# yanzq95/DHD

Hardware: AMD Instinct MI355X
Metric: samples/sec (6-cam fwd+bwd) DHD-S view-transform hot path (higher is better)
Workload: dtype f32

## Files before the change

### dhd_amd/csrc/mghs_layout.h

```cpp
#pragma once
#include "vec16.h"

namespace dhd {

constexpr int kBlock = 256;
constexpr int kScanItems = 8;
constexpr int kChunk = kBlock * kScanItems;
constexpr int kTileC = 64;
constexpr int kCamFloats = 36;
#ifndef DHD_SEG_ROWS
#define DHD_SEG_ROWS 4
#endif
constexpr int kSegRows = DHD_SEG_ROWS;
constexpr int kSegMaxVox = 256 * kSegRows;
constexpr int kMaxTileX = 256;
constexpr int kRowGroup = 4;

struct Layout {
  int B, N, D, fh, fw, C, G;
  int dhw;
  int hw;
  int P;
  int V;
  int R;
  int n_chunks;
  int vox_base[DHD_MAX_GRIDS + 1];
  int row_base[DHD_MAX_GRIDS + 1];
  dhd_grid grid[DHD_MAX_GRIDS];
  int compact;
  int n_slots_max;
  int n_segs;
  int seg_base[DHD_MAX_GRIDS + 1];
  int nxc;
  int sched_heavy, sched_ratio;
  int flags;
  int columns;
  int* count;
  unsigned long long* scan_state;
  int* offset;
  int* key;
  int* rnk;
  int4* s_ent;
  float* cam;
  float* dg_part;
  float* fg_stage;
  float* vsum;
  int* nzoff;
  int* nzvox;
  int* p_slot;
  size_t zero_bytes;
};

inline size_t align_up(size_t v, size_t a) { return (v + a - 1) / a * a; }

__host__ __device__ inline int pt_natural(const Layout& L, int bn, int d, int h, int w) { return bn * L.dhw + (d * L.fh + h) * L.fw + w; }
__host__ __device__ inline int pt_index(const Layout& L, int bn, int d, int h, int w) {
#ifdef DHD_KEYS_ROWMAJOR
  return pt_natural(L, bn, d, h, w);
#else
  return bn * L.dhw + (d * L.fw + w) * L.fh + h;
#endif
}

inline int make_layout(const dhd_mghs_desc* d, const dhd_mghs_workspace* ws, Layout* L, size_t* state_bytes = nullptr,
                       size_t* scratch_bytes = nullptr) {
  if (!d) return DHD_EINVAL;
  if (d->batch <= 0 || d->n_cams <= 0 || d->n_depth <= 0 || d->fh <= 0 || d->fw <= 0 || d->channels <= 0)
    return DHD_EINVAL;
  if (d->n_grids < 1 || d->n_grids > DHD_MAX_GRIDS) return DHD_EINVAL;
  if (d->flags & ~(DHD_MGHS_DETERMINISTIC | DHD_MGHS_FEAT_GRAD_NCHW | DHD_MGHS_DEBUG_SCAN_SELF_SERVE)) return DHD_EINVAL;
  L->flags = d->flags;
  L->B = d->batch; L->N = d->n_cams; L->D = d->n_depth; L->fh = d->fh; L->fw = d->fw;
  L->C = d->channels; L->G = d->n_grids;
  L->hw = d->fh * d->fw;
  long dhw = (long)d->n_depth * L->hw;
  long P = (long)d->batch * d->n_cams * dhw;
  if (P > (1L << 29)) return DHD_EUNSUPPORTED;
  L->dhw = (int)dhw; L->P = (int)P;
  long v = 0, r = 0;
  bool compact = d->channels == kTileC;
  int nx_max = 0;
  for (int g = 0; g < DHD_MAX_GRIDS; ++g) {
    L->vox_base[g] = (int)v; L->row_base[g] = (int)r; L->seg_base[g] = (int)(r / kSegRows);
    if (g < d->n_grids) {
      const dhd_grid& gr = d->grid[g];
      if (gr.n[0] <= 0 || gr.n[1] <= 0 || gr.n[2] <= 0) return DHD_EINVAL;
      L->grid[g] = gr;
      v += (long)d->batch * gr.n[2] * gr.n[1] * gr.n[0];
      r += (long)d->batch * gr.n[2] * gr.n[1];
      if (v > (1L << 30)) return DHD_EUNSUPPORTED;
      compact = compact && gr.n[1] % kSegRows == 0 && gr.n[0] % 4 == 0 && gr.n[0] * kSegRows <= kSegMaxVox;
      nx_max = nx_max > gr.n[0] ? nx_max : gr.n[0];
    } else {
      L->grid[g] = d->grid[0];
    }
  }
  L->vox_base[DHD_MAX_GRIDS] = (int)v; L->row_base[DHD_MAX_GRIDS] = (int)r;
  for (int g = d->n_grids; g < DHD_MAX_GRIDS; ++g) { L->vox_base[g] = (int)v; L->row_base[g] = (int)r; }
  L->V = (int)v; L->R = (int)r;
  L->compact = compact ? 1 : 0;
  L->columns = (compact && d->n_grids > 1 && !(d->flags & DHD_MGHS_DETERMINISTIC) && d->fh == 32) ? 1 : 0;
  L->n_segs = compact ? (int)(r / kSegRows) : 0;
  for (int g = d->n_grids; g <= DHD_MAX_GRIDS; ++g) L->seg_base[g] = (int)(r / kSegRows);
  L->n_chunks = dhd_cdiv(v, kChunk);
  L->nxc = (nx_max + kMaxTileX - 1) / kMaxTileX;
  L->sched_heavy = 0; L->sched_ratio = 0;
  if (L->G > 1 && L->row_base[1] % kRowGroup == 0) {
    int heavy = L->row_base[1] / kRowGroup, light = (L->R - L->row_base[1]) / kRowGroup;
    int k = heavy > 0 ? light / heavy : 0;
    if (k > 4) k = 4;
    if (k == 3) k = 2;
    if (k == 1) k = 0;
    if (k >= 2) { L->sched_heavy = heavy; L->sched_ratio = k; }
  }
  if (ws) {
    if (!ws->state || !ws->scratch) return DHD_EINVAL;
    if ((reinterpret_cast<uintptr_t>(ws->state) | reinterpret_cast<uintptr_t>(ws->scratch)) & 255) return DHD_EINVAL;
  }
  const size_t P2 = 2 * (size_t)L->P;
  const size_t v0 = (size_t)L->vox_base[1], vb = (size_t)L->V - v0, pp = (size_t)L->P;
  const size_t max_slots = (v0 < pp ? v0 : pp) + (vb < pp ? vb : pp);
  L->n_slots_max = (int)max_slots;
  size_t off = 0;
  char* base = ws ? static_cast<char*>(ws->scratch) : nullptr;
  auto carve = [&](size_t n_words) { int* p = reinterpret_cast<int*>(base + off); off = align_up(off + n_words * 4, 256); return p; };
  L->count = carve((size_t)L->V);
  L->scan_state = reinterpret_cast<unsigned long long*>(carve(2 * (size_t)L->n_chunks));
  L->zero_bytes = off;
  if (compact) L->offset = carve((size_t)L->V + 1);
  L->key = carve(P2);
  L->rnk = carve(P2);
  if (compact) L->s_ent = reinterpret_cast<int4*>(carve(4 * P2));
  L->cam = reinterpret_cast<float*>(carve((size_t)L->B * L->N * kCamFloats));
  L->dg_part = reinterpret_cast<float*>(carve(compact ? 0 : P2));
  L->fg_stage = reinterpret_cast<float*>(carve(compact ? 0 : (size_t)L->B * L->N * L->hw * L->C));
  L->vsum = reinterpret_cast<float*>(carve(compact ? (max_slots + 1) * kTileC : 0));
  const size_t scratch_need = off;
  off = 0;
  base = ws ? static_cast<char*>(ws->state) : nullptr;
  L->nzoff = carve((size_t)L->V + 1);
  L->nzvox = carve(max_slots);
  L->p_slot = carve(P2);
  if (!compact) {
    L->offset = carve((size_t)L->V + 1);
    L->s_ent = reinterpret_cast<int4*>(carve(4 * P2));
  }
  const size_t state_need = off;
  if (state_bytes) *state_bytes = state_need;
  if (scratch_bytes) *scratch_bytes = scratch_need;
  if (ws && (ws->state_bytes < state_need || ws->scratch_bytes < scratch_need)) return DHD_ENOSPACE;
  return DHD_OK;
}

__device__ __forceinline__ int rfl(int v) { return __builtin_amdgcn_readfirstlane(v); }
__device__ __forceinline__ int lane_i(int v, int l) { return __builtin_amdgcn_readlane(v, l); }
__device__ __forceinline__ float lane_f(float v, int l) {
  return __int_as_float(__builtin_amdgcn_readlane(__float_as_int(v), l));
}
__device__ __forceinline__ int wave_sum_i(int v) {
  for (int m = 32; m > 0; m >>= 1) v += __shfl_xor(v, m, DHD_WAVE);
  return v;
}

struct OutPtrs { float* p[DHD_MAX_GRIDS]; long sb[DHD_MAX_GRIDS], sz[DHD_MAX_GRIDS], sc[DHD_MAX_GRIDS]; int dtype; };
struct InPtrs { const float* p[DHD_MAX_GRIDS]; long sb[DHD_MAX_GRIDS], sz[DHD_MAX_GRIDS], sc[DHD_MAX_GRIDS]; int dtype; };

template <class Ptrs, class T>
inline int make_views(const Layout& L, T* const bases[DHD_MAX_GRIDS], const dhd_tensor_view* views, Ptrs* o) {
  o->dtype = DHD_F32;
  if (views) {
    o->dtype = views[0].dtype;
    if (o->dtype != DHD_F32 && o->dtype != DHD_F16 && o->dtype != DHD_BF16) return DHD_EINVAL;
    if (o->dtype != DHD_F32 && !L.compact) return DHD_EUNSUPPORTED;
  }
  const long vec = o->dtype == DHD_F32 ? 4 : 8;
  for (int g = 0; g < DHD_MAX_GRIDS; ++g) {
    o->p[g] = nullptr; o->sb[g] = o->sz[g] = o->sc[g] = 0;
    if (g >= L.G) continue;
    const long plane = (long)L.grid[g].n[1] * L.grid[g].n[0];
    if (views) {
      if (!views[g].ptr) return DHD_EINVAL;
      o->p[g] = static_cast<T*>(const_cast<void*>(static_cast<const void*>(views[g].ptr)));
      o->sb[g] = views[g].batch_stride; o->sz[g] = views[g].z_stride; o->sc[g] = views[g].channel_stride;
      if (views[g].dtype != o->dtype) return DHD_EINVAL;
      if (((o->sb[g] | o->sz[g] | o->sc[g]) & (vec - 1)) || (reinterpret_cast<uintptr_t>(views[g].ptr) & 15)) return DHD_EINVAL;
      if (o->dtype != DHD_F32 && (L.grid[g].n[0] & 1)) return DHD_EUNSUPPORTED;
    } else {
      if (!bases || !bases[g]) return DHD_EINVAL;
      if (reinterpret_cast<uintptr_t>(bases[g]) & 15) return DHD_EINVAL;
      o->p[g] = bases[g];
      o->sb[g] = (long)L.grid[g].n[2] * L.C * plane; o->sz[g] = (long)L.C * plane; o->sc[g] = plane;
    }
  }
  return DHD_OK;
}

int launch_scan(const Layout& L, hipStream_t st);
int launch_stream_fwd(const Layout& L, const OutPtrs& o, int split, hipStream_t st, bool op = false);
int launch_stream_bwd(const Layout& L, const InPtrs& in, int split, hipStream_t st, bool op = false);

}
```

### dhd_amd/csrc/mghs_pool.hip

```cpp
#include "lift_device.h"
#include <stdlib.h>
#include "mghs_layout.h"

namespace dhd {
namespace {

#ifndef DHD_STREAM_BLOCK
#define DHD_STREAM_BLOCK 512
#endif
constexpr int kStreamBlock = DHD_STREAM_BLOCK;
constexpr int kStreamWaves = kStreamBlock / DHD_WAVE;
#ifndef DHD_TABLE_FLOATS
#define DHD_TABLE_FLOATS 8192
#endif
constexpr int kTableFloats = DHD_TABLE_FLOATS;

struct Segment {
  int g, b, z, y0, nx, ny, nz;
  int v0;
  int nvox;
};

__device__ __forceinline__ bool decode_segment(const Layout& L, int s, Segment* sg) {
  if (s >= L.n_segs) return false;
  int g = 0;
#pragma unroll
  for (int k = 1; k < DHD_MAX_GRIDS; ++k)
    if (k < L.G && s >= L.seg_base[k]) g = k;
  const dhd_grid& gr = L.grid[g];
  const int local = s - L.seg_base[g];
  const int per_plane = gr.n[1] / kSegRows;
  sg->g = g; sg->nx = gr.n[0]; sg->ny = gr.n[1]; sg->nz = gr.n[2];
  sg->y0 = (local % per_plane) * kSegRows;
  const int bz = local / per_plane;
  sg->z = bz % gr.n[2];
  sg->b = bz / gr.n[2];
  sg->nvox = kSegRows * gr.n[0];
  sg->v0 = L.vox_base[g] + local * sg->nvox;
  return true;
}

__device__ __forceinline__ int channels_per_pass(int nnz) {
  int cp = kTileC;
  while (cp > 4 && (nnz | 1) * cp > kTableFloats) cp >>= 1;
  return cp;
}

template <int J>
struct GatherStep {
  static __device__ __forceinline__ void load(float (&f)[DHD_WAVE], __amdgpu_buffer_rsrc_t feat_rsrc, int lane4, int pix,
                                              int jmax) {
    if ((J & 7) == 0 && J > jmax) return;
    f[J] = __int_as_float(__builtin_amdgcn_raw_buffer_load_b32(feat_rsrc, lane4, lane_i(pix, J) << 8, 0));
    GatherStep<J + 1>::load(f, feat_rsrc, lane4, pix, jmax);
  }
  static __device__ __forceinline__ void run(const float (&f)[DHD_WAVE], unsigned long long firsts, int term, int slot,
                                             float dv, float* vrow, int scratch_row, int jmax, int& cur, float& acc) {
    if ((J & 7) == 0 && J > jmax) return;
    if ((firsts >> J) & 1ull) {
      vrow[(size_t)cur * kTileC] = acc;
      cur = rfl((J == term) ? scratch_row : lane_i(slot, J));
      acc = 0.f;
    }
    acc = fmaf(lane_f(dv, J), f[J], acc);
    GatherStep<J + 1>::run(f, firsts, term, slot, dv, vrow, scratch_row, jmax, cur, acc);
  }
};
template <>
struct GatherStep<DHD_WAVE> {
  static __device__ __forceinline__ void load(float (&)[DHD_WAVE], __amdgpu_buffer_rsrc_t, int, int, int) {}
  static __device__ __forceinline__ void run(const float (&)[DHD_WAVE], unsigned long long, int, int, float, float*, int, int,
                                             int&, float&) {}
};

template <bool BANDS_ONLY>
__device__ __forceinline__ void gather_sums_body(const Layout& L, const float* __restrict__ depth, const float* __restrict__ feat,
                                                 const int block) {
  const int lane = threadIdx.x & 63;
  const int T0 = BANDS_ONLY ? L.offset[L.vox_base[1]] : 0;
  const int T = L.offset[L.V];
  const int per_xcd = ((T - T0 + kBlock - 1) / kBlock + 7) >> 3;
  if ((block >> 3) >= per_xcd) return;
  const int wg = (block & 7) * per_xcd + (block >> 3);
  const int a = rfl(T0 + (wg * (kBlock / DHD_WAVE) + (threadIdx.x >> 6)) * DHD_WAVE);
  if (a >= T) return;
  const int b = min(T, a + DHD_WAVE);
  const __amdgpu_buffer_rsrc_t feat_rsrc = __builtin_amdgcn_make_buffer_rsrc(
      const_cast<float*>(feat), 0, L.B * L.N * L.hw * kTileC * 4, 0x00020000);
  const int lane4 = 4 * lane;
  const int scratch_row = L.n_slots_max;
  float* vrow = L.vsum + lane;
  bool started = false;
  int cur = rfl(scratch_row);
  float acc = 0.f;
  int idx = a + lane;
  int slot_n = -1, prev_n = -2, pix_n = 0, pid_n = 0;
  float dv_n = 0.f;
  if (idx < T) {
    const int4 en = L.s_ent[idx];
    slot_n = en.z;
    pix_n = en.y;
    pid_n = en.x;
    if (idx > T0) prev_n = L.s_ent[idx - 1].z;
  }
  if (idx < T) dv_n = depth[pid_n];
  for (int a0 = a; a0 < T; a0 += DHD_WAVE) {
    const int nb = min(DHD_WAVE, T - a0);
    const int slot = slot_n, pix = pix_n;
    const float dv = dv_n;
    unsigned long long firsts = __ballot(lane < nb && slot != prev_n);
    int lo = 0;
    if (!started) {
      if (firsts == 0ull) lo = nb;
      else lo = __builtin_ctzll(firsts);
      if (a0 + lo >= b) break;
      started = lo < nb;
    }
    int term = DHD_WAVE;
    {
      const int s = min(max(b - a0, lo + 1), DHD_WAVE);
      const unsigned long long m = s >= DHD_WAVE ? 0ull : (firsts >> s) << s;
      if (m != 0ull) term = __builtin_ctzll(m);
      else if (nb < DHD_WAVE) term = nb;
    }
    const bool last = term < DHD_WAVE;
    if (last) firsts = (firsts & ((1ull << term) - 1ull)) | (1ull << term);
    if (lo >= nb) firsts = 0ull;
    idx = a0 + DHD_WAVE + lane;
    slot_n = -1; pix_n = 0; pid_n = 0;
    if (!last && idx < T) {
      const int4 en = L.s_ent[idx];
      slot_n = en.z;
      pix_n = en.y;
      pid_n = en.x;
      prev_n = L.s_ent[idx - 1].z;
    }
    if (lo < nb) {
      const int jmax = last ? term : DHD_WAVE - 1;
      float f[DHD_WAVE];
      GatherStep<0>::load(f, feat_rsrc, lane4, pix, jmax);
      GatherStep<0>::run(f, firsts, term, slot, dv, vrow, scratch_row, jmax, cur, acc);
    }
    if (last) { cur = rfl(scratch_row); break; }
    dv_n = 0.f;
    if (idx < T) dv_n = depth[pid_n];
  }
  vrow[(size_t)cur * kTileC] = acc;
}

template <bool BANDS_ONLY>
__global__ __launch_bounds__(kBlock) void mghs_gather_sums(Layout L, const float* __restrict__ depth,
                                                            const float* __restrict__ feat) {
  gather_sums_body<BANDS_ONLY>(L, depth, feat, (int)blockIdx.x);
}

constexpr int kDepthChunk = 8;

__global__ __launch_bounds__(kBlock) void mghs_zero_grid0_rows(Layout L) {
  const int n0 = L.nzoff[L.vox_base[1]];
  f32x4* v = reinterpret_cast<f32x4*>(L.vsum);
  const size_t n4 = (size_t)n0 * (kTileC / 4);
  const f32x4 z = {0.f, 0.f, 0.f, 0.f};
  for (size_t i = (size_t)blockIdx.x * kBlock + threadIdx.x; i < n4; i += (size_t)gridDim.x * kBlock) v[i] = z;
}

template <int FH, int H>
struct ColStep {
  static __device__ __forceinline__ void run(const float (&f)[FH], unsigned long long firsts, int slot, float dv, float* vrow,
                                             int& cur, float& acc) {
    if ((firsts >> H) & 1ull) {
      if (cur >= 0) atomicAdd(vrow + (size_t)cur * kTileC, acc);
      cur = rfl(lane_i(slot, H));
      acc = 0.f;
    }
    acc = fmaf(lane_f(dv, H), f[H], acc);
    ColStep<FH, H + 1>::run(f, firsts, slot, dv, vrow, cur, acc);
  }
};
template <int FH>
struct ColStep<FH, FH> {
  static __device__ __forceinline__ void run(const float (&)[FH], unsigned long long, int, float, float*, int&, float&) {}
};

template <int FH>
__device__ __forceinline__ void col_sums_body(const Layout& L, const float* __restrict__ depth, const float* __restrict__ feat,
                                              const int block) {
  const int lane = threadIdx.x & 63;
  const int n_chunks = (L.D + kDepthChunk - 1) / kDepthChunk;
  const int wave = rfl((int)(block * (kBlock / DHD_WAVE) + (threadIdx.x >> 6)));
  const int n_cols = L.B * L.N * L.fw;
  if (wave >= n_cols * n_chunks) return;
  const int chunk = wave / n_cols, col = wave - chunk * n_cols;
  const int bn = col / L.fw, w = col - bn * L.fw;
  float f[FH];
#pragma unroll
  for (int h = 0; h < FH; ++h) f[h] = feat[((size_t)(bn * FH + h) * L.fw + w) * kTileC + lane];
  float* vrow = L.vsum + lane;
  const int d0 = chunk * kDepthChunk;
  const int hl = lane < FH ? lane : FH - 1;
  int key[kDepthChunk], slot[kDepthChunk];
  float dv[kDepthChunk];
#pragma unroll
  for (int k = 0; k < kDepthChunk; ++k) {
    const int d = min(d0 + k, L.D - 1);
    const int p = ((bn * L.D + d) * FH + hl) * L.fw + w;
    key[k] = d0 + k < L.D ? L.key[pt_index(L, bn, d, hl, w)] : -1;
    dv[k] = depth[p];
  }
#pragma unroll
  for (int k = 0; k < kDepthChunk; ++k) slot[k] = key[k] >= 0 ? L.nzoff[key[k]] : -1;
#pragma unroll
  for (int k = 0; k < kDepthChunk; ++k) {
    const int prev = __shfl_up(slot[k], 1, DHD_WAVE);
    const unsigned long long firsts = __ballot(lane < FH && (lane == 0 || slot[k] != prev));
    const float dvk = key[k] >= 0 ? dv[k] : 0.f;
    int cur = -1;
    float acc = 0.f;
    ColStep<FH, 0>::run(f, firsts, slot[k], dvk, vrow, cur, acc);
    if (cur >= 0) atomicAdd(vrow + (size_t)cur * kTileC, acc);
  }
}

template <int FH>
__global__ __launch_bounds__(kBlock) void mghs_col_sums(Layout L, const float* __restrict__ depth, const float* __restrict__ feat) {
  col_sums_body<FH>(L, depth, feat, (int)blockIdx.x);
}

template <int FH>
__global__ __launch_bounds__(kBlock) void mghs_sums_cols_bands(Layout L, const float* __restrict__ depth, const float* __restrict__ feat,
                                                               int n_col_groups, int n_gather_groups, int kc) {
  const int grp = rfl((int)(blockIdx.x >> 3)), x = (int)(blockIdx.x & 7);
  const int period = grp / (kc + 1), r = grp - (kc + 1) * period;
  if (r < kc) {
    const int cg = kc * period + r;
    if (cg < n_col_groups) col_sums_body<FH>(L, depth, feat, (cg << 3) | x);
  } else if (period < n_gather_groups) {
    gather_sums_body<true>(L, depth, feat, (period << 3) | x);
  }
}

constexpr size_t kStreamLds = (size_t)kTableFloats * 4 + (size_t)kSegMaxVox * 2 + 16;

template <class T> __device__ __forceinline__ f32x4 pack_vox(const float* f) {
  typedef T vox __attribute__((ext_vector_type(kVec16<T>)));
  vox v;
#pragma unroll
  for (int k = 0; k < kVec16<T>; ++k) v[k] = (T)f[k];
  return __builtin_bit_cast(f32x4, v);
}
template <class T> __device__ __forceinline__ void unpack_vox(f32x4 v, float* f) { widen16<T>(__builtin_bit_cast(raw16<T>, v), f); }

template <class T, int OP = 0>
__global__ __launch_bounds__(kStreamBlock) void mghs_stream_fwd(Layout L, OutPtrs out, int split) {
  constexpr int VPL = kVec16<T>;
  extern __shared__ __attribute__((aligned(16))) char smem[];
  float* table = reinterpret_cast<float*>(smem);
  unsigned short* slot_of = reinterpret_cast<unsigned short*>(smem + (size_t)kTableFloats * 4);
  int* ctl = reinterpret_cast<int*>(smem + (size_t)kTableFloats * 4 + (size_t)kSegMaxVox * 2);

  const int seg = blockIdx.x / split, pw = kTileC / split;
  const int c_begin = (blockIdx.x % split) * pw, c_end = c_begin + pw;
  Segment sg;
  if (!decode_segment(L, seg, &sg)) return;
  const int t = threadIdx.x, lane = t & 63, wv = t >> 6;
  if (t == 0) ctl[0] = L.nzoff[sg.v0];
  if (t == 1) ctl[1] = L.nzoff[sg.v0 + sg.nvox];
  for (int i = t; i < kSegMaxVox / 2; i += kStreamBlock) reinterpret_cast<unsigned*>(slot_of)[i] = 0u;
  __syncthreads();
  const int k0 = rfl(ctl[0]), nnz = rfl(ctl[1]) - k0;
  for (int j = t; j < nnz; j += kStreamBlock) slot_of[L.nzvox[k0 + j] - sg.v0] = (unsigned short)(j + 1);
  const int cp = min(channels_per_pass(nnz), c_end - c_begin), pitch = nnz | 1;
  const int nvec = sg.nvox / VPL;
  T* og = reinterpret_cast<T*>(out.p[sg.g]);
  const long sb = out.sb[sg.g], sz = out.sz[sg.g], sc = out.sc[sg.g];
  for (int c_lo = c_begin; c_lo < c_end; c_lo += cp) {
    __syncthreads();
    for (int i = t; i < nnz * cp; i += kStreamBlock) {
      const int j = i / cp, cc = i % cp;
      table[cc * pitch + j] = L.vsum[(size_t)(k0 + j) * kTileC + c_lo + cc];
    }
    __syncthreads();
    T* base = og + (size_t)sg.b * sb + (size_t)sg.z * sz + (size_t)c_lo * sc + (size_t)sg.y0 * sg.nx;
    const int total = cp * nvec;
    constexpr int kStride = kStreamWaves * DHD_WAVE;
    const int q_step = kStride / nvec, r_step = kStride % nvec;
    int idx = wv * DHD_WAVE + lane;
    int cc = idx / nvec, i = idx % nvec;
    for (; idx < total; idx += kStride) {
      float f[VPL];
#pragma unroll
      for (int k = 0; k < VPL; ++k) f[k] = 0.f;
      unsigned sl[VPL / 2];
      if (VPL == 4) {
        const uint2 w = *reinterpret_cast<const uint2*>(slot_of + 4 * i);
        sl[0] = w.x; sl[1] = w.y;
      } else {
        const uint4 w = *reinterpret_cast<const uint4*>(slot_of + 8 * i);
        sl[0] = w.x; sl[1] = w.y; sl[VPL / 2 - 2] = w.z; sl[VPL / 2 - 1] = w.w;
      }
      unsigned any = 0;
#pragma unroll
      for (int k = 0; k < VPL / 2; ++k) any |= sl[k];
      if (any) {
#pragma unroll
        for (int k = 0; k < VPL / 2; ++k) {
          const unsigned s0 = sl[k] & 0xffffu, s1 = sl[k] >> 16;
          if (s0) f[2 * k] = table[cc * pitch + (s0 - 1)];
          if (s1) f[2 * k + 1] = table[cc * pitch + (s1 - 1)];
        }
      }
      f32x4* dst = reinterpret_cast<f32x4*>(base + (size_t)cc * sc) + i;
      __builtin_nontemporal_store(pack_vox<T>(f), dst);
      cc += q_step;
      i += r_step;
      if (i >= nvec) { i -= nvec; ++cc; }
    }
  }
}

template <class T, int OP = 0>
__global__ __launch_bounds__(kStreamBlock) void mghs_stream_bwd(Layout L, InPtrs og_in, int split) {
  constexpr int VPL = kVec16<T>;
  extern __shared__ __attribute__((aligned(16))) char smem[];
  float* table = reinterpret_cast<float*>(smem);
  unsigned short* slot_of = reinterpret_cast<unsigned short*>(smem + (size_t)kTableFloats * 4);
  int* ctl = reinterpret_cast<int*>(smem + (size_t)kTableFloats * 4 + (size_t)kSegMaxVox * 2);

  const int seg = blockIdx.x / split, pw = kTileC / split;
  const int c_begin = (blockIdx.x % split) * pw, c_end = c_begin + pw;
  Segment sg;
  if (!decode_segment(L, seg, &sg)) return;
  const int t = threadIdx.x, lane = t & 63, wv = t >> 6;
  if (t == 0) ctl[0] = L.nzoff[sg.v0];
  if (t == 1) ctl[1] = L.nzoff[sg.v0 + sg.nvox];
  for (int i = t; i < kSegMaxVox / 2; i += kStreamBlock) reinterpret_cast<unsigned*>(slot_of)[i] = 0u;
  __syncthreads();
  const int k0 = rfl(ctl[0]), nnz = rfl(ctl[1]) - k0;
  if (nnz == 0) return;
  for (int j = t; j < nnz; j += kStreamBlock) slot_of[L.nzvox[k0 + j] - sg.v0] = (unsigned short)(j + 1);
  const int cp = min(channels_per_pass(nnz), c_end - c_begin), pitch = nnz | 1;
  const int nvec = sg.nvox / VPL;
  const T* og = reinterpret_cast<const T*>(og_in.p[sg.g]);
  const long sb = og_in.sb[sg.g], sz = og_in.sz[sg.g], sc = og_in.sc[sg.g];
  constexpr int kStride = kStreamWaves * DHD_WAVE, kBatch = 5;
  const int q_step = kStride / nvec, r_step = kStride % nvec;
  const T* gbase = og + (size_t)sg.b * sb + (size_t)sg.z * sz + (size_t)sg.y0 * sg.nx;
  __syncthreads();
  for (int c_lo = c_begin; c_lo < c_end; c_lo += cp) {
    __syncthreads();
    const int total = cp * nvec;
    int idx = wv * DHD_WAVE + lane;
    int cc = idx / nvec, i = idx % nvec;
    for (; idx - lane < total; ) {
      unsigned sl[kBatch][VPL / 2], any[kBatch];
      f32x4 v[kBatch];
      int ccs[kBatch];
#pragma unroll
      for (int k = 0; k < kBatch; ++k) {
        const bool in = idx < total;
        if (VPL == 4) {
          const uint2 w = in ? *reinterpret_cast<const uint2*>(slot_of + 4 * i) : make_uint2(0u, 0u);
          sl[k][0] = w.x; sl[k][1] = w.y;
        } else {
          const uint4 w = in ? *reinterpret_cast<const uint4*>(slot_of + 8 * i) : make_uint4(0u, 0u, 0u, 0u);
          sl[k][0] = w.x; sl[k][1] = w.y; sl[k][VPL / 2 - 2] = w.z; sl[k][VPL / 2 - 1] = w.w;
        }
        any[k] = 0;
#pragma unroll
        for (int u = 0; u < VPL / 2; ++u) any[k] |= sl[k][u];
        ccs[k] = cc;
        const f32x4* p = any[k] ? reinterpret_cast<const f32x4*>(gbase + (size_t)(c_lo + cc) * sc) + i
                                  : reinterpret_cast<const f32x4*>(L.vsum);
        v[k] = __builtin_nontemporal_load(p);
        idx += kStride;
        cc += q_step;
        i += r_step;
        if (i >= nvec) { i -= nvec; ++cc; }
      }
#pragma unroll
      for (int k = 0; k < kBatch; ++k) {
        if (any[k]) {
          float f[VPL];
          unpack_vox<T>(v[k], f);
#pragma unroll
          for (int u = 0; u < VPL / 2; ++u) {
            const unsigned s0 = sl[k][u] & 0xffffu, s1 = sl[k][u] >> 16;
            if (s0) table[ccs[k] * pitch + (s0 - 1)] = f[2 * u];
            if (s1) table[ccs[k] * pitch + (s1 - 1)] = f[2 * u + 1];
          }
        }
      }
    }
    __syncthreads();
    for (int i = t; i < nnz * cp; i += kStreamBlock) {
      const int j = i / cp, cc = i % cp;
      L.vsum[(size_t)(k0 + j) * kTileC + c_lo + cc] = table[cc * pitch + j];
    }
  }
}

__device__ __forceinline__ float row16_sum(float v) {
  v += __int_as_float(__builtin_amdgcn_update_dpp(0, __float_as_int(v), 0x128, 0xf, 0xf, false));
  v += __int_as_float(__builtin_amdgcn_update_dpp(0, __float_as_int(v), 0x124, 0xf, 0xf, false));
  v += __int_as_float(__builtin_amdgcn_update_dpp(0, __float_as_int(v), 0x122, 0xf, 0xf, false));
  v += __int_as_float(__builtin_amdgcn_update_dpp(0, __float_as_int(v), 0x121, 0xf, 0xf, false));
  return v;
}

__global__ __launch_bounds__(kBlock) void mghs_pixel_bwd(Layout L, const float* __restrict__ depth,
                                                          const float* __restrict__ feat, float* __restrict__ depth_grad,
                                                          float* __restrict__ feat_grad) {
  const int lane = threadIdx.x & 63;
  const int es = lane >> 4, cq = lane & 15;
  const int per_xcd = gridDim.x >> 3;
  const int wg = (blockIdx.x & 7) * per_xcd + (blockIdx.x >> 3);
  const int q = rfl(wg * (kBlock / DHD_WAVE) + (threadIdx.x >> 6));
  if (q >= L.B * L.N * L.hw) return;
  const int bn = q / L.hw, pl = q % L.hw;
  const int p0 = bn * L.dhw + pl;
  const f32x4 f = reinterpret_cast<const f32x4*>(feat)[(size_t)q * (kTileC / 4) + cq];
  const f32x4* gc = reinterpret_cast<const f32x4*>(L.vsum) + cq;
  f32x4 fg = {0.f, 0.f, 0.f, 0.f};
  const int n_cand = 2 * L.D;
  constexpr int kRounds = DHD_WAVE / 4, kU = 8;
  for (int e0 = 0; e0 < n_cand; e0 += DHD_WAVE) {
    const int nb = min(DHD_WAVE, n_cand - e0);
    int slot = -1;
    float dv = 0.f;
    if (lane < nb) {
      const int e = e0 + lane;
      const int pid = p0 + (e >> 1) * L.hw;
      slot = L.p_slot[(e & 1) * L.P + pid];
      dv = depth[pid];
    }
    float mine = 0.f;
#pragma unroll
    for (int u0 = 0; u0 < kRounds; u0 += kU) {
      if (4 * u0 >= nb) break;
      f32x4 g[kU];
      float d[kU];
#pragma unroll
      for (int j = 0; j < kU; ++j) {
        const int i = 4 * (u0 + j) + es;
        const int sl = __shfl(slot, i, DHD_WAVE);
        d[j] = __shfl(dv, i, DHD_WAVE);
        g[j] = sl >= 0 ? gc[(size_t)sl * (kTileC / 4)] : fg * 0.f;
      }
#pragma unroll
      for (int j = 0; j < kU; ++j) {
        fg += g[j] * d[j];
        const float part = row16_sum((g[j].x * f.x + g[j].y * f.y) + (g[j].z * f.z + g[j].w * f.w));
        const float both = part + __shfl_xor(part, 16, DHD_WAVE);
        if (cq == u0 + j) mine = both;
      }
    }
    const int cand = 4 * cq + es;
    if (!(es & 1) && cand < nb) depth_grad[p0 + ((e0 + cand) >> 1) * L.hw] = mine;
  }
#pragma unroll
  for (int c = 0; c < 4; ++c) {
    float v = fg[c];
    v += __shfl_xor(v, 16, DHD_WAVE);
    v += __shfl_xor(v, 32, DHD_WAVE);
    fg[c] = v;
  }
  if (es == 0) {
    if (L.flags & DHD_MGHS_FEAT_GRAD_NCHW) {
      float* dst = feat_grad + ((size_t)bn * kTileC + 4 * cq) * L.hw + pl;
#pragma unroll
      for (int c = 0; c < 4; ++c) dst[(size_t)c * L.hw] = fg[c];
    } else {
      reinterpret_cast<f32x4*>(feat_grad)[(size_t)q * (kTileC / 4) + cq] = fg;
    }
  }
}

__global__ __launch_bounds__(kLiftBlock) void mghs_fg_to_nchw(const float* __restrict__ src, float* __restrict__ dst, int rows, int cols) {
  __shared__ float tile[64][65];
  transpose_tile(tile, src, dst, rows, cols, blockIdx.z, blockIdx.y * 64, blockIdx.x * 64);
}

__global__ __launch_bounds__(kBlock) void mghs_sum_parts(const float* __restrict__ part, int P, float* __restrict__ out) {
  const int i = blockIdx.x * kBlock + threadIdx.x;
  if (i < P) out[i] = part[i] + part[P + i];
}

constexpr int kRowBlock = 512;
constexpr int kRowWaves = kRowBlock / DHD_WAVE;

struct RowTile {
  int g, b, z, y, nx, ny, nz;
  int vrow;
};

__device__ __forceinline__ bool decode_row(const Layout& L, int r, RowTile* t) {
  if (r >= L.R) return false;
  int g = 0;
#pragma unroll
  for (int k = 1; k < DHD_MAX_GRIDS; ++k)
    if (k < L.G && r >= L.row_base[k]) g = k;
  const dhd_grid& gr = L.grid[g];
  int local = r - L.row_base[g];
  t->g = g; t->nx = gr.n[0]; t->ny = gr.n[1]; t->nz = gr.n[2];
  t->y = local % gr.n[1];
  int bz = local / gr.n[1];
  t->z = bz % gr.n[2];
  t->b = bz / gr.n[2];
  t->vrow = L.vox_base[g] + local * gr.n[0];
  return true;
}

__device__ __forceinline__ int scheduled_tile(const Layout& L, int block, int* xchunk) {
  const int pos = xcd_grouped_tile(block, kRowGroup * L.nxc);
  *xchunk = pos % L.nxc;
  const int rpos = pos / L.nxc;
  int grp = rpos / kRowGroup;
  const int within = rpos % kRowGroup;
  if (L.sched_heavy > 0) {
    const int k1 = L.sched_ratio + 1;
    if (grp < L.sched_heavy * k1) {
      const int q = grp / k1, r = grp % k1;
      grp = (r == 0) ? q : L.sched_heavy + q * L.sched_ratio + (r - 1);
    }
  }
  return grp * kRowGroup + within;
}

__global__ __launch_bounds__(kRowBlock) void mghs_rows_fwd(Layout L, const float* __restrict__ depth,
                                                           const float* __restrict__ feat, OutPtrs out, int tile_stride) {
  extern __shared__ __attribute__((aligned(16))) char smem[];
  float* tile = reinterpret_cast<float*>(smem);
  int* offs = reinterpret_cast<int*>(smem + (size_t)kTileC * tile_stride * 4);
  RowTile rt;
  int xchunk;
  if (!decode_row(L, scheduled_tile(L, blockIdx.x, &xchunk), &rt)) return;
  const int c0 = blockIdx.y * kTileC;
  const int cn = min(kTileC, L.C - c0);
  const int x0 = xchunk * kMaxTileX;
  if (x0 >= rt.nx) return;
  const int xn = min(kMaxTileX, rt.nx - x0);
  const int t = threadIdx.x, lane = t & 63, wv = t >> 6;

  for (int i = t; i <= xn; i += kRowBlock) offs[i] = L.offset[rt.vrow + x0 + i];
  for (int i = t; i < cn * tile_stride; i += kRowBlock) tile[i] = 0.f;
  __syncthreads();

  if (offs[xn] != offs[0]) {
    const int CL = next_pow2(cn);
    const int nsub = DHD_WAVE / CL;
    const int c = lane % CL, sub = lane / CL;
    const bool c_ok = c < cn;
    const float* featc = feat + c0 + c;
    for (int x = wv; x < xn; x += kRowWaves) {
      const int s = offs[x], e = offs[x + 1];
      if (e == s) continue;
      float acc = 0.f;
      for (int s0 = s; s0 < e; s0 += DHD_WAVE) {
        const int nb = min(DHD_WAVE, e - s0);
        int pix = 0;
        float dv = 0.f;
        if (lane < nb) {
          const int4 en = L.s_ent[s0 + lane];
          pix = en.y;
          dv = depth[en.x];
        }
        const int steps = (nb + nsub - 1) / nsub;
        for (int k = 0; k < steps; ++k) {
          const int i = k * nsub + sub;
          const bool live = i < nb;
          int q = __shfl(pix, live ? i : 0, DHD_WAVE);
          float d = __shfl(dv, live ? i : 0, DHD_WAVE);
          float f = (live && c_ok) ? featc[(size_t)q * L.C] : 0.f;
          acc = fmaf(d, f, acc);
        }
      }
      for (int m = CL; m < DHD_WAVE; m <<= 1) acc += __shfl_xor(acc, m, DHD_WAVE);
      if (sub == 0 && c_ok) tile[c * tile_stride + x] = acc;
    }
    __syncthreads();
  }

  float* og = out.p[rt.g];
  const bool vec = ((rt.nx & 3) == 0) && ((xn & 3) == 0) && ((x0 & 3) == 0);
  for (int cc = wv; cc < cn; cc += kRowWaves) {
    size_t row = (size_t)rt.b * out.sb[rt.g] + (size_t)rt.z * out.sz[rt.g] + (size_t)(c0 + cc) * out.sc[rt.g] + (size_t)rt.y * rt.nx + x0;
    const float* src = tile + cc * tile_stride;
    if (vec) {
      f32x4* dst = reinterpret_cast<f32x4*>(og + row);
      for (int i = lane; i < xn / 4; i += DHD_WAVE) {
        f32x4 v = {src[4 * i], src[4 * i + 1], src[4 * i + 2], src[4 * i + 3]};
        __builtin_nontemporal_store(v, dst + i);
      }
    } else {
      for (int i = lane; i < xn; i += DHD_WAVE) __builtin_nontemporal_store(src[i], og + row + i);
    }
  }
}

__global__ __launch_bounds__(kRowBlock) void mghs_rows_bwd(Layout L, const float* __restrict__ depth,
                                                           const float* __restrict__ feat, InPtrs og,
                                                           float* __restrict__ feat_grad, int tile_stride) {
  extern __shared__ __attribute__((aligned(16))) char smem[];
  float* tile = reinterpret_cast<float*>(smem);
  int* offs = reinterpret_cast<int*>(smem + (size_t)kTileC * tile_stride * 4);
  RowTile rt;
  int xchunk;
  if (!decode_row(L, scheduled_tile(L, blockIdx.x, &xchunk), &rt)) return;
  const int c0 = blockIdx.y * kTileC;
  const int cn = min(kTileC, L.C - c0);
  const int x0 = xchunk * kMaxTileX;
  if (x0 >= rt.nx) return;
  const int xn = min(kMaxTileX, rt.nx - x0);
  const int t = threadIdx.x, lane = t & 63, wv = t >> 6;

  for (int i = t; i <= xn; i += kRowBlock) offs[i] = L.offset[rt.vrow + x0 + i];
  __syncthreads();
  if (offs[xn] == offs[0]) return;

  const float* gsrc = og.p[rt.g];
  const bool vec = ((rt.nx & 3) == 0) && ((xn & 3) == 0) && ((x0 & 3) == 0);
  for (int cc = wv; cc < cn; cc += kRowWaves) {
    size_t row = (size_t)rt.b * og.sb[rt.g] + (size_t)rt.z * og.sz[rt.g] + (size_t)(c0 + cc) * og.sc[rt.g] + (size_t)rt.y * rt.nx + x0;
    float* dst = tile + cc * tile_stride;
    if (vec) {
      const float4* src = reinterpret_cast<const float4*>(gsrc + row);
      for (int i = lane; i < xn / 4; i += DHD_WAVE) {
        float4 v = src[i];
        dst[4 * i] = v.x; dst[4 * i + 1] = v.y; dst[4 * i + 2] = v.z; dst[4 * i + 3] = v.w;
      }
    } else {
      for (int i = lane; i < xn; i += DHD_WAVE) dst[i] = gsrc[row + i];
    }
  }
  __syncthreads();

  float* dgp = L.dg_part + (rt.g == 0 ? 0 : L.P);
  const bool dg_atomic = L.C > kTileC;
  const int CL = next_pow2(cn);
  const int nsub = DHD_WAVE / CL;
  const int c = lane % CL, sub = lane / CL;
  const bool c_ok = c < cn;
  const float* featc = feat + c0 + c;
  float* fgc = feat_grad + c0 + c;
  for (int x = wv; x < xn; x += kRowWaves) {
    const int s = offs[x], e = offs[x + 1];
    if (e == s) continue;
    const float g = c_ok ? tile[c * tile_stride + x] : 0.f;
    for (int s0 = s; s0 < e; s0 += DHD_WAVE) {
      const int nb = min(DHD_WAVE, e - s0);
      int pix = 0, pid = 0;
      float dv = 0.f;
      if (lane < nb) {
        const int4 en = L.s_ent[s0 + lane];
        pix = en.y;
        pid = en.x;
        dv = depth[pid];
      }
      float mine = 0.f;
      const int steps = (nb + nsub - 1) / nsub;
      for (int k = 0; k < steps; ++k) {
        const int i = k * nsub + sub;
        const bool live = i < nb;
        int q = __shfl(pix, live ? i : 0, DHD_WAVE);
        float d = __shfl(dv, live ? i : 0, DHD_WAVE);
        float prod = 0.f;
        if (live && c_ok) {
          float f = featc[(size_t)q * L.C];
          unsafeAtomicAdd(fgc + (size_t)q * L.C, g * d);
          prod = g * f;
        }
        float tot = group_sum(prod, CL);
        int owner_sub = lane - k * nsub;
        float got = __shfl(tot, (owner_sub >= 0 && owner_sub < nsub) ? owner_sub * CL : 0, DHD_WAVE);
        if (owner_sub >= 0 && owner_sub < nsub) mine = got;
      }
      if (lane < nb) {
        if (dg_atomic) unsafeAtomicAdd(dgp + pid, mine); else dgp[pid] = mine;
      }
    }
  }
}

void rows_launch_shape(const Layout& L, int* stride, size_t* smem, dim3* grid) {
  int nx_max = 0;
  for (int g = 0; g < L.G; ++g) nx_max = nx_max > L.grid[g].n[0] ? nx_max : L.grid[g].n[0];
  int xt = nx_max < kMaxTileX ? nx_max : kMaxTileX;
  *stride = xt | 1;
  *smem = (size_t)kTileC * (*stride) * 4 + (size_t)(kMaxTileX + 1) * 4;
  *grid = dim3(xcd_grouped_blocks(L.R * L.nxc, kRowGroup * L.nxc), dhd_cdiv(L.C, kTileC), 1);
}

}

int launch_stream_fwd(const Layout& L, const OutPtrs& o, int split, hipStream_t st, bool op) {
  if (!L.compact || L.n_segs <= 0) return DHD_EINVAL;
  if (op) {
    if (o.dtype != DHD_F32) return DHD_EUNSUPPORTED;
    hipLaunchKernelGGL((mghs_stream_fwd<float, 1>), dim3(L.n_segs * split), dim3(kStreamBlock), kStreamLds, st, L, o, split);
    DHD_LAUNCH_CHECK();
    return DHD_OK;
  }
  return with_dtype<NativeHalf>(o.dtype, [&](auto* t) {
    hipLaunchKernelGGL(mghs_stream_fwd<std::remove_pointer_t<decltype(t)>>, dim3(L.n_segs * split), dim3(kStreamBlock), kStreamLds, st, L, o, split);
    DHD_LAUNCH_CHECK();
    return DHD_OK;
  });
}

int launch_stream_bwd(const Layout& L, const InPtrs& in, int split, hipStream_t st, bool op) {
  if (!L.compact || L.n_segs <= 0) return DHD_EINVAL;
  if (op) {
    if (in.dtype != DHD_F32) return DHD_EUNSUPPORTED;
    hipLaunchKernelGGL((mghs_stream_bwd<float, 1>), dim3(L.n_segs * split), dim3(kStreamBlock), kStreamLds, st, L, in, split);
    DHD_LAUNCH_CHECK();
    return DHD_OK;
  }
  return with_dtype<NativeHalf>(in.dtype, [&](auto* t) {
    hipLaunchKernelGGL(mghs_stream_bwd<std::remove_pointer_t<decltype(t)>>, dim3(L.n_segs * split), dim3(kStreamBlock), kStreamLds, st, L, in, split);
    DHD_LAUNCH_CHECK();
    return DHD_OK;
  });
}

}

using namespace dhd;

static int stream_split(const Layout& L) {
  return (long)L.P < 300L * L.n_segs ? 4 : 2;
}

extern "C" {

int dhd_mghs_forward_gather(const dhd_mghs_desc* desc, const float* depth, const float* feat_nhwc, const dhd_mghs_workspace* workspace,
                            void* stream) {
  Layout L;
  int rc = make_layout(desc, workspace, &L);
  if (rc) return rc;
  if (!workspace || !depth || !feat_nhwc) return DHD_EINVAL;
  if (L.compact && !dhd_aligned(16, feat_nhwc)) return DHD_EINVAL;
  if (!L.compact) return DHD_OK;
  hipStream_t st = dhd_stream(stream);
  if (L.columns) {
    hipLaunchKernelGGL(mghs_zero_grid0_rows, dim3(1024), dim3(kBlock), 0, st, L);
    const int waves = L.B * L.N * L.fw * dhd_cdiv(L.D, kDepthChunk);
    const dim3 grid(dhd_cdiv(waves, kBlock / DHD_WAVE));
    const int n_gather = dhd_cdiv((long)L.P, 8 * kBlock) * 8;
    static const bool merged = getenv("DHD_MGHS_SEPARATE_SUMS") == nullptr;
    constexpr int kc = 2;
    if (merged) {
      const int ncg = dhd_cdiv(grid.x, 8), ngg = n_gather / 8;
      const int periods = ((ncg + kc - 1) / kc) > ngg ? (ncg + kc - 1) / kc : ngg;
      hipLaunchKernelGGL(mghs_sums_cols_bands<32>, dim3(periods * (kc + 1) * 8), dim3(kBlock), 0, st, L, depth, feat_nhwc, ncg, ngg, kc);
    } else {
      hipLaunchKernelGGL(mghs_col_sums<32>, grid, dim3(kBlock), 0, st, L, depth, feat_nhwc);
      hipLaunchKernelGGL(mghs_gather_sums<true>, dim3(n_gather), dim3(kBlock), 0, st, L, depth, feat_nhwc);
    }
  } else {
    hipLaunchKernelGGL(mghs_gather_sums<false>, dim3(dhd_cdiv(2L * L.P, 8 * kBlock) * 8), dim3(kBlock), 0, st, L, depth, feat_nhwc);
  }
  DHD_LAUNCH_CHECK();
  return DHD_OK;
}

static int forward_stream_impl(const dhd_mghs_desc* desc, const float* depth, const float* feat_nhwc,
                               float* const out[DHD_MAX_GRIDS], const dhd_tensor_view* views, const dhd_mghs_workspace* workspace,
                               void* stream) {
  Layout L;
  int rc = make_layout(desc, workspace, &L);
  if (rc) return rc;
  if (!workspace || !depth || !feat_nhwc || (!out && !views)) return DHD_EINVAL;
  if (L.compact && !dhd_aligned(16, feat_nhwc)) return DHD_EINVAL;
  OutPtrs o;
  if ((rc = make_views<OutPtrs, float>(L, out, views, &o))) return rc;
  hipStream_t st = dhd_stream(stream);
  if (L.compact) {
    if ((rc = launch_stream_fwd(L, o, o.dtype == DHD_F32 ? stream_split(L) : 2, st))) return rc;
  } else {
    int stride; size_t smem; dim3 grid;
    rows_launch_shape(L, &stride, &smem, &grid);
    hipLaunchKernelGGL(mghs_rows_fwd, grid, dim3(kRowBlock), smem, st, L, depth, feat_nhwc, o, stride);
    DHD_LAUNCH_CHECK();
  }
  return DHD_OK;
}

int dhd_mghs_forward_stream(const dhd_mghs_desc* desc, const float* depth, const float* feat_nhwc,
                            float* const out[DHD_MAX_GRIDS], const dhd_mghs_workspace* workspace, void* stream) {
  return forward_stream_impl(desc, depth, feat_nhwc, out, nullptr, workspace, stream);
}

int dhd_mghs_forward_stream_views(const dhd_mghs_desc* desc, const float* depth, const float* feat_nhwc,
                                  const dhd_tensor_view out[DHD_MAX_GRIDS], const dhd_mghs_workspace* workspace, void* stream) {
  if (!out) return DHD_EINVAL;
  return forward_stream_impl(desc, depth, feat_nhwc, nullptr, out, workspace, stream);
}

int dhd_mghs_forward(const dhd_mghs_desc* desc, const float* depth, const float* feat_nhwc,
                     float* const out[DHD_MAX_GRIDS], const dhd_mghs_workspace* workspace, void* stream) {
  int rc = dhd_mghs_forward_gather(desc, depth, feat_nhwc, workspace, stream);
  if (rc) return rc;
  return forward_stream_impl(desc, depth, feat_nhwc, out, nullptr, workspace, stream);
}

int dhd_mghs_forward_views(const dhd_mghs_desc* desc, const float* depth, const float* feat_nhwc,
                           const dhd_tensor_view out[DHD_MAX_GRIDS], const dhd_mghs_workspace* workspace, void* stream) {
  if (!out) return DHD_EINVAL;
  int rc = dhd_mghs_forward_gather(desc, depth, feat_nhwc, workspace, stream);
  if (rc) return rc;
  return forward_stream_impl(desc, depth, feat_nhwc, nullptr, out, workspace, stream);
}

static int backward_impl(const dhd_mghs_desc* desc, const float* depth, const float* feat_nhwc,
                         const float* const out_grad[DHD_MAX_GRIDS], const dhd_tensor_view* views, float* depth_grad,
                         float* feat_grad_nhwc, const dhd_mghs_workspace* workspace, void* stream) {
  Layout L;
  int rc = make_layout(desc, workspace, &L);
  if (rc) return rc;
  if (!workspace || !depth || !feat_nhwc || (!out_grad && !views) || !depth_grad || !feat_grad_nhwc) return DHD_EINVAL;
  if (L.compact && !dhd_aligned(16, feat_nhwc, feat_grad_nhwc)) return DHD_EINVAL;
  InPtrs in;
  if ((rc = make_views<InPtrs, const float>(L, out_grad, views, &in))) return rc;
  hipStream_t st = dhd_stream(stream);
  if (L.compact) {
    if ((rc = launch_stream_bwd(L, in, stream_split(L) == 2 ? 2 : 1, st))) return rc;
    hipLaunchKernelGGL(mghs_pixel_bwd, dim3(dhd_cdiv((long)L.B * L.N * L.hw, 8 * (kBlock / DHD_WAVE)) * 8), dim3(kBlock), 0, st, L,
                       depth, feat_nhwc, depth_grad, feat_grad_nhwc);
    DHD_LAUNCH_CHECK();
    return DHD_OK;
  }
  const bool to_nchw = (L.flags & DHD_MGHS_FEAT_GRAD_NCHW) != 0;
  float* fg = to_nchw ? L.fg_stage : feat_grad_nhwc;
  DHD_HIP(hipMemsetAsync(L.dg_part, 0, 2 * (size_t)L.P * 4, st));
  DHD_HIP(hipMemsetAsync(fg, 0, (size_t)L.B * L.N * L.hw * L.C * 4, st));
  int stride; size_t smem; dim3 grid;
  rows_launch_shape(L, &stride, &smem, &grid);
  hipLaunchKernelGGL(mghs_rows_bwd, grid, dim3(kRowBlock), smem, st, L, depth, feat_nhwc, in, fg, stride);
  DHD_LAUNCH_CHECK();
  if (to_nchw) {
    hipLaunchKernelGGL(mghs_fg_to_nchw, dim3(dhd_cdiv(L.C, 64), dhd_cdiv(L.hw, 64), L.B * L.N), dim3(kLiftBlock), 0, st, fg,
                       feat_grad_nhwc, L.hw, L.C);
    DHD_LAUNCH_CHECK();
  }
  hipLaunchKernelGGL(mghs_sum_parts, dim3(dhd_cdiv(L.P, kBlock)), dim3(kBlock), 0, st, L.dg_part, L.P, depth_grad);
  DHD_LAUNCH_CHECK();
  return DHD_OK;
}

int dhd_mghs_backward(const dhd_mghs_desc* desc, const float* depth, const float* feat_nhwc,
                      const float* const out_grad[DHD_MAX_GRIDS], float* depth_grad, float* feat_grad_nhwc,
                      const dhd_mghs_workspace* workspace, void* stream) {
  return backward_impl(desc, depth, feat_nhwc, out_grad, nullptr, depth_grad, feat_grad_nhwc, workspace, stream);
}

int dhd_mghs_backward_views(const dhd_mghs_desc* desc, const float* depth, const float* feat_nhwc,
                            const dhd_tensor_view out_grad[DHD_MAX_GRIDS], float* depth_grad, float* feat_grad_nhwc,
                            const dhd_mghs_workspace* workspace, void* stream) {
  if (!out_grad) return DHD_EINVAL;
  return backward_impl(desc, depth, feat_nhwc, nullptr, out_grad, depth_grad, feat_grad_nhwc, workspace, stream);
}

}
```

Measured before the change: 2768.

## Overlap band-grid streaming with grid-0 gather sums in a merged forward kernel

Adds a by-grid forward path. It first gathers band-grid sums, then runs one merged kernel whose workgroups are split proportionally between streaming the band segments and computing grid-0 gather sums. A final launch streams the grid-0 segments. The goal is to overlap the two independent phases and avoid a full serial gather-then-stream dependency. The gather inner loop can also load features in two halves to lower register pressure in the merged kernel. This adds a third launch and mixed-role workgroups that may cut occupancy because of the stream kernel's LDS use. The path is on by default but is not used when the columns path is active.

```diff
diff --git a/dhd_amd/csrc/mghs_layout.h b/dhd_amd/csrc/mghs_layout.h
--- a/dhd_amd/csrc/mghs_layout.h
+++ b/dhd_amd/csrc/mghs_layout.h
@@ -62,6 +62,16 @@
 #endif
 }
 
+struct RoleSlot { int point, index; };
+__host__ __device__ inline RoleSlot role_of_group(int g, int n_stream, int n_point) {
+  const long long n = (long long)n_stream + n_point;
+  const int before = (int)((long long)g * n_point / n), upto = (int)((long long)(g + 1) * n_point / n);
+  RoleSlot r;
+  r.point = upto > before ? 1 : 0;
+  r.index = r.point ? before : g - before;
+  return r;
+}
+
 inline int make_layout(const dhd_mghs_desc* d, const dhd_mghs_workspace* ws, Layout* L, size_t* state_bytes = nullptr,
                        size_t* scratch_bytes = nullptr) {
   if (!d) return DHD_EINVAL;
diff --git a/dhd_amd/csrc/mghs_pool.hip b/dhd_amd/csrc/mghs_pool.hip
--- a/dhd_amd/csrc/mghs_pool.hip
+++ b/dhd_amd/csrc/mghs_pool.hip
@@ -46,15 +46,15 @@
   return cp;
 }
 
-template <int J>
+template <int J, int END, int N>
 struct GatherStep {
-  static __device__ __forceinline__ void load(float (&f)[DHD_WAVE], __amdgpu_buffer_rsrc_t feat_rsrc, int lane4, int pix,
+  static __device__ __forceinline__ void load(float (&f)[N], __amdgpu_buffer_rsrc_t feat_rsrc, int lane4, int pix,
                                               int jmax) {
     if ((J & 7) == 0 && J > jmax) return;
-    f[J] = __int_as_float(__builtin_amdgcn_raw_buffer_load_b32(feat_rsrc, lane4, lane_i(pix, J) << 8, 0));
-    GatherStep<J + 1>::load(f, feat_rsrc, lane4, pix, jmax);
-  }
-  static __device__ __forceinline__ void run(const float (&f)[DHD_WAVE], unsigned long long firsts, int term, int slot,
+    f[J & (N - 1)] = __int_as_float(__builtin_amdgcn_raw_buffer_load_b32(feat_rsrc, lane4, lane_i(pix, J) << 8, 0));
+    GatherStep<J + 1, END, N>::load(f, feat_rsrc, lane4, pix, jmax);
+  }
+  static __device__ __forceinline__ void run(const float (&f)[N], unsigned long long firsts, int term, int slot,
                                              float dv, float* vrow, int scratch_row, int jmax, int& cur, float& acc) {
     if ((J & 7) == 0 && J > jmax) return;
     if ((firsts >> J) & 1ull) {
@@ -62,27 +62,28 @@
       cur = rfl((J == term) ? scratch_row : lane_i(slot, J));
       acc = 0.f;
     }
-    acc = fmaf(lane_f(dv, J), f[J], acc);
-    GatherStep<J + 1>::run(f, firsts, term, slot, dv, vrow, scratch_row, jmax, cur, acc);
+    acc = fmaf(lane_f(dv, J), f[J & (N - 1)], acc);
+    GatherStep<J + 1, END, N>::run(f, firsts, term, slot, dv, vrow, scratch_row, jmax, cur, acc);
   }
 };
-template <>
-struct GatherStep<DHD_WAVE> {
-  static __device__ __forceinline__ void load(float (&)[DHD_WAVE], __amdgpu_buffer_rsrc_t, int, int, int) {}
-  static __device__ __forceinline__ void run(const float (&)[DHD_WAVE], unsigned long long, int, int, float, float*, int, int,
+template <int END, int N>
+struct GatherStep<END, END, N> {
+  static __device__ __forceinline__ void load(float (&)[N], __amdgpu_buffer_rsrc_t, int, int, int) {}
+  static __device__ __forceinline__ void run(const float (&)[N], unsigned long long, int, int, float, float*, int, int,
                                              int&, float&) {}
 };
 
-template <bool BANDS_ONLY>
+enum { kAllGrids = 0, kBandsOnly = 1, kGrid0Only = 2 };
+template <int PART, bool HALF = false>
 __device__ __forceinline__ void gather_sums_body(const Layout& L, const float* __restrict__ depth, const float* __restrict__ feat,
-                                                 const int block) {
+                                                 const int block, const int wib) {
   const int lane = threadIdx.x & 63;
-  const int T0 = BANDS_ONLY ? L.offset[L.vox_base[1]] : 0;
-  const int T = L.offset[L.V];
+  const int T0 = PART == kBandsOnly ? L.offset[L.vox_base[1]] : 0;
+  const int T = PART == kGrid0Only ? L.offset[L.vox_base[1]] : L.offset[L.V];
   const int per_xcd = ((T - T0 + kBlock - 1) / kBlock + 7) >> 3;
   if ((block >> 3) >= per_xcd) return;
   const int wg = (block & 7) * per_xcd + (block >> 3);
-  const int a = rfl(T0 + (wg * (kBlock / DHD_WAVE) + (threadIdx.x >> 6)) * DHD_WAVE);
+  const int a = rfl(T0 + (wg * (kBlock / DHD_WAVE) + wib) * DHD_WAVE);
   if (a >= T) return;
   const int b = min(T, a + DHD_WAVE);
   const __amdgpu_buffer_rsrc_t feat_rsrc = __builtin_amdgcn_make_buffer_rsrc(
@@ -137,9 +138,18 @@
     }
     if (lo < nb) {
       const int jmax = last ? term : DHD_WAVE - 1;
-      float f[DHD_WAVE];
-      GatherStep<0>::load(f, feat_rsrc, lane4, pix, jmax);
-      GatherStep<0>::run(f, firsts, term, slot, dv, vrow, scratch_row, jmax, cur, acc);
+      if (HALF) {
+        constexpr int H = DHD_WAVE / 2;
+        float f[H];
+        GatherStep<0, H, H>::load(f, feat_rsrc, lane4, pix, jmax);
+        GatherStep<0, H, H>::run(f, firsts, term, slot, dv, vrow, scratch_row, jmax, cur, acc);
+        GatherStep<H, DHD_WAVE, H>::load(f, feat_rsrc, lane4, pix, jmax);
+        GatherStep<H, DHD_WAVE, H>::run(f, firsts, term, slot, dv, vrow, scratch_row, jmax, cur, acc);
+      } else {
+        float f[DHD_WAVE];
+        GatherStep<0, DHD_WAVE, DHD_WAVE>::load(f, feat_rsrc, lane4, pix, jmax);
+        GatherStep<0, DHD_WAVE, DHD_WAVE>::run(f, firsts, term, slot, dv, vrow, scratch_row, jmax, cur, acc);
+      }
     }
     if (last) { cur = rfl(scratch_row); break; }
     dv_n = 0.f;
@@ -148,10 +158,10 @@
   vrow[(size_t)cur * kTileC] = acc;
 }
 
-template <bool BANDS_ONLY>
+template <int PART>
 __global__ __launch_bounds__(kBlock) void mghs_gather_sums(Layout L, const float* __restrict__ depth,
                                                             const float* __restrict__ feat) {
-  gather_sums_body<BANDS_ONLY>(L, depth, feat, (int)blockIdx.x);
+  gather_sums_body<PART>(L, depth, feat, (int)blockIdx.x, (int)(threadIdx.x >> 6));
 }
 
 constexpr int kDepthChunk = 8;
@@ -235,7 +245,7 @@
     const int cg = kc * period + r;
     if (cg < n_col_groups) col_sums_body<FH>(L, depth, feat, (cg << 3) | x);
   } else if (period < n_gather_groups) {
-    gather_sums_body<true>(L, depth, feat, (period << 3) | x);
+    gather_sums_body<kBandsOnly>(L, depth, feat, (period << 3) | x, (int)(threadIdx.x >> 6));
   }
 }
 
@@ -250,18 +260,19 @@
 }
 template <class T> __device__ __forceinline__ void unpack_vox(f32x4 v, float* f) { widen16<T>(__builtin_bit_cast(raw16<T>, v), f); }
 
-template <class T, int OP = 0>
-__global__ __launch_bounds__(kStreamBlock) void mghs_stream_fwd(Layout L, OutPtrs out, int split) {
+template <class T>
+__device__ __forceinline__ void stream_fwd_body(const Layout& L, const OutPtrs& out, const int split, const int wg, const int seg_lo,
+                                                const int seg_hi) {
   constexpr int VPL = kVec16<T>;
   extern __shared__ __attribute__((aligned(16))) char smem[];
   float* table = reinterpret_cast<float*>(smem);
   unsigned short* slot_of = reinterpret_cast<unsigned short*>(smem + (size_t)kTableFloats * 4);
   int* ctl = reinterpret_cast<int*>(smem + (size_t)kTableFloats * 4 + (size_t)kSegMaxVox * 2);
 
-  const int seg = blockIdx.x / split, pw = kTileC / split;
-  const int c_begin = (blockIdx.x % split) * pw, c_end = c_begin + pw;
+  const int seg = seg_lo + wg / split, pw = kTileC / split;
+  const int c_begin = (wg % split) * pw, c_end = c_begin + pw;
   Segment sg;
-  if (!decode_segment(L, seg, &sg)) return;
+  if (seg >= seg_hi || !decode_segment(L, seg, &sg)) return;
   const int t = threadIdx.x, lane = t & 63, wv = t >> 6;
   if (t == 0) ctl[0] = L.nzoff[sg.v0];
   if (t == 1) ctl[1] = L.nzoff[sg.v0 + sg.nvox];
@@ -315,6 +326,34 @@
       i += r_step;
       if (i >= nvec) { i -= nvec; ++cc; }
     }
+  }
+}
+
+template <class T, int OP = 0>
+__global__ __launch_bounds__(kStreamBlock) void mghs_stream_fwd(Layout L, OutPtrs out, int split, int seg_lo, int seg_hi) {
+  stream_fwd_body<T>(L, out, split, (int)blockIdx.x, seg_lo, seg_hi);
+}
+
+#ifndef DHD_MERGED_GATHER_HALF
+#define DHD_MERGED_GATHER_HALF 1
+#endif
+#ifndef DHD_MERGED_WAVES
+#define DHD_MERGED_WAVES 8
+#endif
+constexpr int kPointPerStream = kStreamBlock / kBlock;
+
+template <class T>
+__global__ __launch_bounds__(kStreamBlock, DHD_MERGED_WAVES) void mghs_fwd_bands_g0sums(Layout L, OutPtrs out, int split,
+                                                                                        const float* __restrict__ depth,
+                                                                                        const float* __restrict__ feat,
+                                                                                        int n_stream_groups, int n_point_groups) {
+  const int grp = rfl((int)(blockIdx.x >> 3)), x = (int)(blockIdx.x & 7);
+  const RoleSlot r = role_of_group(grp, n_stream_groups, n_point_groups);
+  if (r.point) {
+    const int block = ((kPointPerStream * r.index + (int)(threadIdx.x / kBlock)) << 3) | x;
+    gather_sums_body<kGrid0Only, DHD_MERGED_GATHER_HALF != 0>(L, depth, feat, block, (int)(threadIdx.x % kBlock) >> 6);
+  } else {
+    stream_fwd_body<T>(L, out, split, (r.index << 3) | x, L.seg_base[1], L.n_segs);
   }
 }
 
@@ -696,12 +735,12 @@
   if (!L.compact || L.n_segs <= 0) return DHD_EINVAL;
   if (op) {
     if (o.dtype != DHD_F32) return DHD_EUNSUPPORTED;
-    hipLaunchKernelGGL((mghs_stream_fwd<float, 1>), dim3(L.n_segs * split), dim3(kStreamBlock), kStreamLds, st, L, o, split);
+    hipLaunchKernelGGL((mghs_stream_fwd<float, 1>), dim3(L.n_segs * split), dim3(kStreamBlock), kStreamLds, st, L, o, split, 0, L.n_segs);
     DHD_LAUNCH_CHECK();
     return DHD_OK;
   }
   return with_dtype<NativeHalf>(o.dtype, [&](auto* t) {
-    hipLaunchKernelGGL(mghs_stream_fwd<std::remove_pointer_t<decltype(t)>>, dim3(L.n_segs * split), dim3(kStreamBlock), kStreamLds, st, L, o, split);
+    hipLaunchKernelGGL(mghs_stream_fwd<std::remove_pointer_t<decltype(t)>>, dim3(L.n_segs * split), dim3(kStreamBlock), kStreamLds, st, L, o, split, 0, L.n_segs);
     DHD_LAUNCH_CHECK();
     return DHD_OK;
   });
@@ -754,10 +793,10 @@
       hipLaunchKernelGGL(mghs_sums_cols_bands<32>, dim3(periods * (kc + 1) * 8), dim3(kBlock), 0, st, L, depth, feat_nhwc, ncg, ngg, kc);
     } else {
       hipLaunchKernelGGL(mghs_col_sums<32>, grid, dim3(kBlock), 0, st, L, depth, feat_nhwc);
-      hipLaunchKernelGGL(mghs_gather_sums<true>, dim3(n_gather), dim3(kBlock), 0, st, L, depth, feat_nhwc);
+      hipLaunchKernelGGL(mghs_gather_sums<kBandsOnly>, dim3(n_gather), dim3(kBlock), 0, st, L, depth, feat_nhwc);
     }
   } else {
-    hipLaunchKernelGGL(mghs_gather_sums<false>, dim3(dhd_cdiv(2L * L.P, 8 * kBlock) * 8), dim3(kBlock), 0, st, L, depth, feat_nhwc);
+    hipLaunchKernelGGL(mghs_gather_sums<kAllGrids>, dim3(dhd_cdiv(2L * L.P, 8 * kBlock) * 8), dim3(kBlock), 0, st, L, depth, feat_nhwc);
   }
   DHD_LAUNCH_CHECK();
   return DHD_OK;
@@ -796,19 +835,65 @@
   return forward_stream_impl(desc, depth, feat_nhwc, nullptr, out, workspace, stream);
 }
 
+enum { kByGridForward = 1, kByGridBackward = 2 };
+static int by_grid(const Layout& L) {
+  static const int env = [] {
+    const char* s = getenv("DHD_MGHS_BY_GRID");
+    return s && *s ? atoi(s) & (kByGridForward | kByGridBackward) : kByGridForward;
+  }();
+  return L.compact && L.G > 1 && !L.columns ? env : 0;
+}
+
+static int forward_by_grid(const Layout& L, const float* depth, const float* feat_nhwc, const OutPtrs& o, hipStream_t st) {
+  const int split = o.dtype == DHD_F32 ? stream_split(L) : 2;
+  const int n_gather = dhd_cdiv((long)L.P, 8 * kBlock) * 8;
+  hipLaunchKernelGGL(mghs_gather_sums<kBandsOnly>, dim3(n_gather), dim3(kBlock), 0, st, L, depth, feat_nhwc);
+  DHD_LAUNCH_CHECK();
+  const int n_stream = dhd_cdiv((long)(L.n_segs - L.seg_base[1]) * split, 8L);
+  const int n_point = dhd_cdiv((long)(n_gather / 8), (long)kPointPerStream);
+  if (n_stream + n_point > 0) {
+    int rc = with_dtype<NativeHalf>(o.dtype, [&](auto* t) {
+      hipLaunchKernelGGL(mghs_fwd_bands_g0sums<std::remove_pointer_t<decltype(t)>>, dim3((n_stream + n_point) * 8), dim3(kStreamBlock), kStreamLds,
+                         st, L, o, split, depth, feat_nhwc, n_stream, n_point);
+      DHD_LAUNCH_CHECK();
+      return DHD_OK;
+    });
+    if (rc) return rc;
+  }
+  if (L.seg_base[1] <= 0) return DHD_OK;
+  return with_dtype<NativeHalf>(o.dtype, [&](auto* t) {
+    hipLaunchKernelGGL((mghs_stream_fwd<std::remove_pointer_t<decltype(t)>, 2>), dim3(L.seg_base[1] * split), dim3(kStreamBlock), kStreamLds, st,
+                       L, o, split, 0, L.seg_base[1]);
+    DHD_LAUNCH_CHECK();
+    return DHD_OK;
+  });
+}
+
+static int forward_impl(const dhd_mghs_desc* desc, const float* depth, const float* feat_nhwc, float* const out[DHD_MAX_GRIDS],
+                        const dhd_tensor_view* views, const dhd_mghs_workspace* workspace, void* stream) {
+  Layout L;
+  int rc = make_layout(desc, workspace, &L);
+  if (rc) return rc;
+  if (by_grid(L) & kByGridForward) {
+    if (!workspace || !depth || !feat_nhwc || (!out && !views)) return DHD_EINVAL;
+    if (!dhd_aligned(16, feat_nhwc)) return DHD_EINVAL;
+    OutPtrs o;
+    if ((rc = make_views<OutPtrs, float>(L, out, views, &o))) return rc;
+    return forward_by_grid(L, depth, feat_nhwc, o, dhd_stream(stream));
+  }
+  if ((rc = dhd_mghs_forward_gather(desc, depth, feat_nhwc, workspace, stream))) return rc;
+  return forward_stream_impl(desc, depth, feat_nhwc, out, views, workspace, stream);
+}
+
 int dhd_mghs_forward(const dhd_mghs_desc* desc, const float* depth, const float* feat_nhwc,
                      float* const out[DHD_MAX_GRIDS], const dhd_mghs_workspace* workspace, void* stream) {
-  int rc = dhd_mghs_forward_gather(desc, depth, feat_nhwc, workspace, stream);
-  if (rc) return rc;
-  return forward_stream_impl(desc, depth, feat_nhwc, out, nullptr, workspace, stream);
+  return forward_impl(desc, depth, feat_nhwc, out, nullptr, workspace, stream);
 }
 
 int dhd_mghs_forward_views(const dhd_mghs_desc* desc, const float* depth, const float* feat_nhwc,
                            const dhd_tensor_view out[DHD_MAX_GRIDS], const dhd_mghs_workspace* workspace, void* stream) {
   if (!out) return DHD_EINVAL;
-  int rc = dhd_mghs_forward_gather(desc, depth, feat_nhwc, workspace, stream);
-  if (rc) return rc;
-  return forward_stream_impl(desc, depth, feat_nhwc, nullptr, out, workspace, stream);
+  return forward_impl(desc, depth, feat_nhwc, nullptr, out, workspace, stream);
 }
 
 static int backward_impl(const dhd_mghs_desc* desc, const float* depth, const float* feat_nhwc,
```

Result: faster. 2805 (median of 6 runs) (+1.3%).
